# AnjieCheng/SpatialRGPT

Measured on NVIDIA H100. Metric: generated_tokens_per_sec, higher is better.
Workload: dtype bf16

## Files before the change

spatialrgpt_b200/csrc/gemv.cu:

```cuda
#include <stdlib.h>

#include "common.cuh"
#include "pack12.cuh"
#include "srgpt_b200.h"

namespace srgpt {
namespace gemv {

constexpr int THREADS = 256;
constexpr int WARPS = THREADS / 32;
constexpr int SPRE_MAX = 2;
constexpr int SPRE_WARP_BYTES = 2 * 4 * 32 * 16;
constexpr int SPRE_WARP_BYTES12 = 2 * 3 * 32 * 16;
enum { MODE_LM = 3 };

struct Params {
  const bf16* x;
  const bf16* W;
  int ldw;
  bf16* y;
  int N, K;
  const bf16* norm_weight;
  float eps;
  const bf16* residual;
  int n_heads, n_kv_heads, hd;
  const bf16* cos_tab;
  const bf16* sin_tab;
  const int* pos;
  bf16* kv_pages;
  const int* page_table;
  int page_size;
  float* logits_out;
  float* part_val;
  int* part_idx;
  unsigned long long* trace;
  int spre;
  int l2pf;
  int kv_heads_total;
  int kv_head_off;
  float* y_f32;
  srgpt_packed12 pk;
};

__device__ __forceinline__ void pdl_launch_dependents() { asm volatile("griddepcontrol.launch_dependents;" ::: "memory"); }
__device__ __forceinline__ void pdl_wait() { asm volatile("griddepcontrol.wait;" ::: "memory"); }

__device__ __forceinline__ void stage_x(const bf16* __restrict__ x, const bf16* __restrict__ norm_weight, float eps, int K,
                                        bf16* sx, float* red, const uint4* nw_pre, bool nw_pre_valid) {
  const int nchunk = K >> 3;
  if (norm_weight == nullptr) {
    for (int c = threadIdx.x; c < nchunk; c += THREADS)
      reinterpret_cast<uint4*>(sx)[c] = reinterpret_cast<const uint4*>(x)[c];
  } else if (nw_pre_valid) {
    uint4 xr[2];
    float sq = 0.f;
#pragma unroll
    for (int k = 0; k < 2; ++k) {
      const int c = threadIdx.x + k * THREADS;
      xr[k] = make_uint4(0, 0, 0, 0);
      if (c < nchunk) xr[k] = reinterpret_cast<const uint4*>(x)[c];
      float f[8];
      unpack8(xr[k], f);
#pragma unroll
      for (int t = 0; t < 8; ++t) sq += f[t] * f[t];
    }
    const float rstd = rsqrtf(block_sum(sq, red) / (float)K + eps);
#pragma unroll
    for (int k = 0; k < 2; ++k) {
      const int c = threadIdx.x + k * THREADS;
      if (c < nchunk) {
        float f[8], w[8], o[8];
        unpack8(xr[k], f);
        unpack8(nw_pre[k], w);
#pragma unroll
        for (int t = 0; t < 8; ++t) o[t] = w[t] * bf16_round(f[t] * rstd);
        reinterpret_cast<uint4*>(sx)[c] = pack8(o);
      }
    }
  } else {
    float sq = 0.f;
    for (int c = threadIdx.x; c < nchunk; c += THREADS) {
      float f[8];
      unpack8(reinterpret_cast<const uint4*>(x)[c], f);
#pragma unroll
      for (int t = 0; t < 8; ++t) sq += f[t] * f[t];
    }
    const float rstd = rsqrtf(block_sum(sq, red) / (float)K + eps);
    for (int c = threadIdx.x; c < nchunk; c += THREADS) {
      float f[8], w[8], o[8];
      unpack8(reinterpret_cast<const uint4*>(x)[c], f);
      unpack8(reinterpret_cast<const uint4*>(norm_weight)[c], w);
#pragma unroll
      for (int t = 0; t < 8; ++t) o[t] = w[t] * bf16_round(f[t] * rstd);
      reinterpret_cast<uint4*>(sx)[c] = pack8(o);
    }
  }
  __syncthreads();
}

__device__ __forceinline__ float dot8(const uint4& w, const float* xf) {
  float f[8];
  unpack8(w, f);
  float a = 0.f;
#pragma unroll
  for (int t = 0; t < 8; ++t) a = fmaf(f[t], xf[t], a);
  return a;
}

__device__ __forceinline__ bool better(float v, int i, float bv, int bi) { return v > bv || (v == bv && i < bi); }

template <int MODE>
__device__ __forceinline__ void pair_rows(const Params& p, int pi, int& r0, int& r1) {
  if (MODE == SRGPT_GEMV_QKV_ROPE) {
    const int half = p.hd >> 1;
    const int head = pi / half, j = pi - head * half;
    r0 = head * p.hd + j;
    r1 = r0 + half;
  } else {
    r0 = 2 * pi;
    r1 = r0 + 1;
    if (MODE == MODE_LM && r1 >= p.N) r1 = r0;
  }
}

struct Raw12 {
  uint4 s01, s23, e;
};

__device__ __forceinline__ Raw12 ld_raw12(const uint4* sm_lane, const uint4* ex_lane, int b) {
  Raw12 q;
  q.s01 = ld_stream16(sm_lane + b * 64);
  q.s23 = ld_stream16(sm_lane + b * 64 + 32);
  q.e = ld_stream16(ex_lane + b * 32);
  return q;
}

__device__ __forceinline__ void decode_batch(const Raw12& q, uint32_t bp, uint4 (&w)[4]) {
  w[0] = pack12::decode_chunk(q.s01.x, q.s01.y, q.e.x, bp);
  w[1] = pack12::decode_chunk(q.s01.z, q.s01.w, q.e.y, bp);
  w[2] = pack12::decode_chunk(q.s23.x, q.s23.y, q.e.z, bp);
  w[3] = pack12::decode_chunk(q.s23.z, q.s23.w, q.e.w, bp);
}

__device__ __forceinline__ void patch_batch(uint4 (&w)[4], int exc, int n, int& j, int b, int lane) {
  while (j < n) {
    const int v = __shfl_sync(0xffffffffu, exc, j);
    const int col = v >> 8;
    if ((col >> 10) != b) break;
    const int cc = col >> 3, t = col & 7;
    const uint32_t bits = ((cc & 31) == lane) ? (uint32_t)(v & 0xFF) << (7 + 16 * (t & 1)) : 0u;
#pragma unroll
    for (int i = 0; i < 4; ++i) {
      const uint32_t m = (i == ((cc >> 5) & 3)) ? bits : 0u;
      w[i].x |= (t >> 1) == 0 ? m : 0u;
      w[i].y |= (t >> 1) == 1 ? m : 0u;
      w[i].z |= (t >> 1) == 2 ? m : 0u;
      w[i].w |= (t >> 1) == 3 ? m : 0u;
    }
    ++j;
  }
}

struct Rows12 {
  uint32_t bp0, bp1;
  int exc0, exc1;
  int n0, n1;
  int j0, j1;
};

__device__ __forceinline__ void consume12(const Raw12& q0, const Raw12& q1, Rows12& rs, int b, int lane, const uint4* px, float& a0, float& a1) {
  uint4 w0[4], w1[4];
  decode_batch(q0, rs.bp0, w0);
  decode_batch(q1, rs.bp1, w1);
  patch_batch(w0, rs.exc0, rs.n0, rs.j0, b, lane);
  patch_batch(w1, rs.exc1, rs.n1, rs.j1, b, lane);
  const int c = b * 128 + lane;
#pragma unroll
  for (int i = 0; i < 4; ++i) {
    float xf[8];
    unpack8(px[c + 32 * i], xf);
    a0 += dot8(w0[i], xf);
    a1 += dot8(w1[i], xf);
  }
}

template <int MODE, int PRE, bool PACKED>
__global__ void __launch_bounds__(THREADS, PRE == 1 ? 3 : (PRE == 2 ? 2 : 1)) decode_gemv_kernel(const Params p) {
  extern __shared__ __align__(16) uint8_t smem_raw[];
  __shared__ float red[32];
  __shared__ float sv[WARPS];
  __shared__ int si[WARPS];
  bf16* sx = reinterpret_cast<bf16*>(smem_raw);

  const int warp = threadIdx.x >> 5, lane = threadIdx.x & 31;
  trace_mark(p.trace, 0);
  const int npairs = (MODE == MODE_LM) ? ((p.N + 1) >> 1) : (p.N >> 1);
  const int pi = blockIdx.x * WARPS + warp;
  const bool active = pi < npairs;
  int r0 = 0, r1 = 0;
  if (active) pair_rows<MODE>(p, pi, r0, r1);
  const uint4* p0 = reinterpret_cast<const uint4*>(p.W + (size_t)r0 * p.ldw);
  const uint4* p1 = reinterpret_cast<const uint4*>(p.W + (size_t)r1 * p.ldw);
  const uint4* px = reinterpret_cast<const uint4*>(sx);
  const int nchunk = p.K >> 3;
  const int nchunk_all = nchunk;

  constexpr int NPRE = 4 * PRE;
  uint4 u0[NPRE], u1[NPRE];
  int c = lane;
  const bool first_full = !PACKED && active && (c + 32 * (NPRE - 1) < nchunk);
  if (first_full) {
#pragma unroll
    for (int i = 0; i < NPRE; ++i) {
      u0[i] = ld_stream16(p0 + c + 32 * i);
      u1[i] = ld_stream16(p1 + c + 32 * i);
    }
  }
  uint8_t* spre_base = smem_raw + (size_t)p.K * 2 + (size_t)warp * ((size_t)p.spre * (PACKED ? SPRE_WARP_BYTES12 : SPRE_WARP_BYTES));
  int n_spre = 0;
  const int nbatch = p.K >> 10;
  Raw12 q0 = {}, q1 = {};
  Rows12 rs = {};
  const uint4 *sm0 = nullptr, *ex0 = nullptr;
  const int drow_ex = (r1 - r0) * (p.K >> 5);
  if (PACKED && active) {
    sm0 = reinterpret_cast<const uint4*>(p.pk.sm) + (size_t)r0 * (p.K >> 4) + lane;
    ex0 = reinterpret_cast<const uint4*>(p.pk.ex) + (size_t)r0 * (p.K >> 5) + lane;
    q0 = ld_raw12(sm0, ex0, 0);
    q1 = ld_raw12(sm0 + 2 * drow_ex, ex0 + drow_ex, 0);
    for (int b = 0; b < p.spre && 1 + b < nbatch; ++b) {
      const uint32_t d = (uint32_t)__cvta_generic_to_shared(spre_base + b * 6 * 512 + lane * 16);
      const uint4 *s = sm0 + (1 + b) * 64, *e = ex0 + (1 + b) * 32;
      asm volatile("cp.async.cg.shared.global [%0], [%1], 16;" ::"r"(d), "l"(s) : "memory");
      asm volatile("cp.async.cg.shared.global [%0], [%1], 16;" ::"r"(d + 512), "l"(s + 32) : "memory");
      asm volatile("cp.async.cg.shared.global [%0], [%1], 16;" ::"r"(d + 1024), "l"(e) : "memory");
      asm volatile("cp.async.cg.shared.global [%0], [%1], 16;" ::"r"(d + 1536), "l"(s + 2 * drow_ex) : "memory");
      asm volatile("cp.async.cg.shared.global [%0], [%1], 16;" ::"r"(d + 2048), "l"(s + 2 * drow_ex + 32) : "memory");
      asm volatile("cp.async.cg.shared.global [%0], [%1], 16;" ::"r"(d + 2560), "l"(e + drow_ex) : "memory");
      ++n_spre;
    }
    asm volatile("cp.async.commit_group;" ::: "memory");
    const int e0 = p.pk.row_ptr[r0], e1 = p.pk.row_ptr[r1];
    rs.n0 = min(p.pk.row_ptr[r0 + 1] - e0, pack12::MAX_EXC_PER_ROW);
    rs.n1 = min(p.pk.row_ptr[r1 + 1] - e1, pack12::MAX_EXC_PER_ROW);
    if (lane < rs.n0) rs.exc0 = p.pk.exc[e0 + lane];
    if (lane < rs.n1) rs.exc1 = p.pk.exc[e1 + lane];
    rs.bp0 = (uint32_t)p.pk.base[r0] - 1u;
    rs.bp1 = (uint32_t)p.pk.base[r1] - 1u;
  }
  if (first_full) {
    for (int b = 0; b < p.spre; ++b) {
      const int cb = c + 32 * NPRE + 128 * b;
      if (cb + 96 >= nchunk) break;
#pragma unroll
      for (int i = 0; i < 4; ++i) {
        const uint32_t d0 = (uint32_t)__cvta_generic_to_shared(spre_base + ((b * 2 + 0) * 4 + i) * 512 + lane * 16);
        const uint32_t d1 = (uint32_t)__cvta_generic_to_shared(spre_base + ((b * 2 + 1) * 4 + i) * 512 + lane * 16);
        asm volatile("cp.async.cg.shared.global [%0], [%1], 16;" ::"r"(d0), "l"(p0 + cb + 32 * i) : "memory");
        asm volatile("cp.async.cg.shared.global [%0], [%1], 16;" ::"r"(d1), "l"(p1 + cb + 32 * i) : "memory");
      }
      ++n_spre;
    }
    asm volatile("cp.async.commit_group;" ::: "memory");
  }
  if (!PACKED && p.l2pf && active && lane < 2) {
    const int c_req = first_full ? (32 * NPRE + 128 * n_spre) : 0;
    if (c_req < nchunk) {
      const char* rowp = reinterpret_cast<const char*>(lane == 0 ? p0 : p1) + (size_t)c_req * 16;
      uint32_t bytes = (uint32_t)(nchunk - c_req) * 16u;
      while (bytes > 0) {
        const uint32_t n = bytes > 16384u ? 16384u : bytes;
        asm volatile("cp.async.bulk.prefetch.L2.global [%0], %1;" ::"l"(rowp), "r"(n) : "memory");
        rowp += n;
        bytes -= n;
      }
    }
  }
  uint4 nw_pre[2] = {make_uint4(0, 0, 0, 0), make_uint4(0, 0, 0, 0)};
  const bool nw_pre_valid = (p.norm_weight != nullptr) && (nchunk_all <= 2 * THREADS);
  if (nw_pre_valid) {
#pragma unroll
    for (int k = 0; k < 2; ++k) {
      const int cc = threadIdx.x + k * THREADS;
      if (cc < nchunk_all) nw_pre[k] = reinterpret_cast<const uint4*>(p.norm_weight)[cc];
    }
  }
  pdl_launch_dependents();
  pdl_wait();
  trace_mark(p.trace, 1);

  stage_x(p.x, p.norm_weight, p.eps, p.K, sx, red, nw_pre, nw_pre_valid);

  float a0 = 0.f, a1 = 0.f;
  if constexpr (PACKED) {
    if (active) {
      consume12(q0, q1, rs, 0, lane, px, a0, a1);
      if (n_spre > 0) {
        asm volatile("cp.async.wait_group 0;" ::: "memory");
        for (int b = 0; b < n_spre; ++b) {
          const uint8_t* s = spre_base + b * 6 * 512 + lane * 16;
          const Raw12 t0 = {*reinterpret_cast<const uint4*>(s), *reinterpret_cast<const uint4*>(s + 512), *reinterpret_cast<const uint4*>(s + 1024)};
          const Raw12 t1 = {*reinterpret_cast<const uint4*>(s + 1536), *reinterpret_cast<const uint4*>(s + 2048), *reinterpret_cast<const uint4*>(s + 2560)};
          consume12(t0, t1, rs, 1 + b, lane, px, a0, a1);
        }
      }
      for (int b = 1 + n_spre; b < nbatch; ++b) {
        const Raw12 t0 = ld_raw12(sm0, ex0, b), t1 = ld_raw12(sm0 + 2 * drow_ex, ex0 + drow_ex, b);
        consume12(t0, t1, rs, b, lane, px, a0, a1);
      }
    }
  } else if (active) {
    if (first_full) {
#pragma unroll
      for (int i = 0; i < NPRE; ++i) {
        float xf[8];
        unpack8(px[c + 32 * i], xf);
        a0 += dot8(u0[i], xf);
        a1 += dot8(u1[i], xf);
      }
      c += 32 * NPRE;
      if (n_spre > 0) {
        asm volatile("cp.async.wait_group 0;" ::: "memory");
        for (int b = 0; b < n_spre; ++b) {
#pragma unroll
          for (int i = 0; i < 4; ++i) {
            float xf[8];
            unpack8(px[c + 32 * i], xf);
            const uint4 w0 = *reinterpret_cast<const uint4*>(spre_base + ((b * 2 + 0) * 4 + i) * 512 + lane * 16);
            const uint4 w1 = *reinterpret_cast<const uint4*>(spre_base + ((b * 2 + 1) * 4 + i) * 512 + lane * 16);
            a0 += dot8(w0, xf);
            a1 += dot8(w1, xf);
          }
          c += 128;
        }
      }
    }
    for (; c + 96 < nchunk; c += 128) {
#pragma unroll
      for (int i = 0; i < 4; ++i) {
        u0[i] = ld_stream16(p0 + c + 32 * i);
        u1[i] = ld_stream16(p1 + c + 32 * i);
      }
#pragma unroll
      for (int i = 0; i < 4; ++i) {
        float xf[8];
        unpack8(px[c + 32 * i], xf);
        a0 += dot8(u0[i], xf);
        a1 += dot8(u1[i], xf);
      }
    }
    for (; c < nchunk; c += 32) {
      float xf[8];
      unpack8(px[c], xf);
      a0 += dot8(ld_stream16(p0 + c), xf);
      a1 += dot8(ld_stream16(p1 + c), xf);
    }
  }
  a0 = warp_sum(a0);
  a1 = warp_sum(a1);
  float best = -INFINITY;
  int besti = 0x7fffffff;
  if (active && lane == 0) {
    if (MODE == SRGPT_GEMV_PLAIN && p.y_f32 != nullptr) {
      *reinterpret_cast<float2*>(p.y_f32 + r0) = make_float2(a0, a1);
    } else if (MODE == SRGPT_GEMV_PLAIN) {
      float y0 = bf16_round(a0), y1 = bf16_round(a1);
      if (p.residual != nullptr) {
        y0 += e2f(p.residual[r0]);
        y1 += e2f(p.residual[r1]);
      }
      *reinterpret_cast<uint32_t*>(p.y + r0) = pack_bf16x2(y0, y1);
    } else if (MODE == SRGPT_GEMV_SWIGLU) {
      const float g = bf16_round(a0), u = bf16_round(a1);
      p.y[pi] = f2e(bf16_round(silu(g)) * u);
    } else if (MODE == SRGPT_GEMV_QKV_ROPE) {
      const int half = p.hd >> 1;
      const int head = pi / half, j = pi - head * half;
      float v0 = bf16_round(a0), v1 = bf16_round(a1);
      const int pos = *p.pos;
      if (head < p.n_heads + p.n_kv_heads) {
        const float cs = e2f(p.cos_tab[(size_t)pos * half + j]);
        const float sn = e2f(p.sin_tab[(size_t)pos * half + j]);
        const float o0 = bf16_round(bf16_round(v0 * cs) + bf16_round(-v1 * sn));
        const float o1 = bf16_round(bf16_round(v1 * cs) + bf16_round(v0 * sn));
        v0 = o0;
        v1 = o1;
      }
      if (head < p.n_heads) {
        p.y[r0] = f2e(v0);
        p.y[r1] = f2e(v1);
      } else {
        const int page = p.page_table[pos / p.page_size], slot = pos % p.page_size;
        const bool is_v = head >= p.n_heads + p.n_kv_heads;
        const int kh = head - p.n_heads - (is_v ? p.n_kv_heads : 0) + p.kv_head_off;
        const int kv_row = (p.kv_heads_total > 0 ? p.kv_heads_total : p.n_kv_heads) * p.hd;
        bf16* dst = p.kv_pages + (((size_t)page * 2 + (is_v ? 1 : 0)) * p.page_size + slot) * kv_row + kh * p.hd;
        dst[j] = f2e(v0);
        dst[j + half] = f2e(v1);
      }
    } else {
      a0 = bf16_round(a0);
      a1 = bf16_round(a1);
      if (p.logits_out != nullptr) {
        p.logits_out[r0] = a0;
        if (r1 != r0) p.logits_out[r1] = a1;
      }
      best = a0;
      besti = r0;
      if (r1 != r0 && better(a1, r1, best, besti)) { best = a1; besti = r1; }
    }
  }
  if (MODE == MODE_LM) {
    if (lane == 0) { sv[warp] = best; si[warp] = besti; }
    __syncthreads();
    if (threadIdx.x == 0) {
      for (int w = 1; w < WARPS; ++w)
        if (better(sv[w], si[w], best, besti)) { best = sv[w]; besti = si[w]; }
      p.part_val[blockIdx.x] = best;
      p.part_idx[blockIdx.x] = besti;
    }
  }
  trace_mark(p.trace, 2);
}

__global__ void __launch_bounds__(256)
lm_head_finalize_kernel(const float* __restrict__ part_val, const int* __restrict__ part_idx, int nparts,
                        const bf16* __restrict__ embed_table, bf16* __restrict__ next_x, int K, long long* __restrict__ out_ids,
                        int* step, int* pos) {
  __shared__ float sv[8];
  __shared__ int si[8];
  __shared__ int s_tok;
  pdl_launch_dependents();
  pdl_wait();
  float best = -INFINITY;
  int bi = 0x7fffffff;
  for (int i = threadIdx.x; i < nparts; i += blockDim.x)
    if (better(part_val[i], part_idx[i], best, bi)) { best = part_val[i]; bi = part_idx[i]; }
#pragma unroll
  for (int o = 16; o > 0; o >>= 1) {
    const float ov = __shfl_xor_sync(0xffffffffu, best, o);
    const int oi = __shfl_xor_sync(0xffffffffu, bi, o);
    if (better(ov, oi, best, bi)) { best = ov; bi = oi; }
  }
  if ((threadIdx.x & 31) == 0) { sv[threadIdx.x >> 5] = best; si[threadIdx.x >> 5] = bi; }
  __syncthreads();
  if (threadIdx.x == 0) {
    for (int w = 1; w < 8; ++w)
      if (better(sv[w], si[w], best, bi)) { best = sv[w]; bi = si[w]; }
    if (bi == 0x7fffffff) bi = 0;
    s_tok = bi;
    out_ids[*step] = (long long)bi;
  }
  __syncthreads();
  const int tok = s_tok;
  if (embed_table != nullptr && next_x != nullptr) {
    const uint4* src = reinterpret_cast<const uint4*>(embed_table + (size_t)tok * K);
    for (int c = threadIdx.x; c < (K >> 3); c += blockDim.x) reinterpret_cast<uint4*>(next_x)[c] = src[c];
  }
  __syncthreads();
  if (threadIdx.x == 0) {
    *step += 1;
    *pos += 1;
  }
}

constexpr int MT_MAX = SRGPT_SPEC_T_MAX;
constexpr int MT_TILE_CH = 512;

struct MParams {
  Params p;
  int T;
  int ldx, ldy;
  int tile_ch;
};

template <int MODE, bool PACKED>
__global__ void __launch_bounds__(THREADS, 2) decode_gemv_multi_kernel(const MParams mp) {
  extern __shared__ __align__(16) uint8_t smem_raw[];
  __shared__ float red[32];
  __shared__ float sv[MT_MAX][WARPS];
  __shared__ int si[MT_MAX][WARPS];
  const Params& p = mp.p;
  const int nt = mp.T, tile_ch = mp.tile_ch;
  bf16* sx = reinterpret_cast<bf16*>(smem_raw);
  const uint4* px = reinterpret_cast<const uint4*>(sx);

  const int warp = threadIdx.x >> 5, lane = threadIdx.x & 31;
  const int npairs = (MODE == MODE_LM) ? ((p.N + 1) >> 1) : (p.N >> 1);
  const int pi = blockIdx.x * WARPS + warp;
  const bool active = pi < npairs;
  int r0 = 0, r1 = 0;
  if (active) pair_rows<MODE>(p, pi, r0, r1);
  const int nchunk = p.K >> 3;
  const int nbatch = (nchunk + 127) >> 7;

  const uint4* p0 = reinterpret_cast<const uint4*>(p.W + (size_t)r0 * p.ldw);
  const uint4* p1 = reinterpret_cast<const uint4*>(p.W + (size_t)r1 * p.ldw);
  uint4 u0[4], u1[4];
  Raw12 q0 = {}, q1 = {};
  Rows12 rs = {};
  const uint4 *sm0 = nullptr, *ex0 = nullptr;
  const int drow_ex = (r1 - r0) * (p.K >> 5);
  auto load_plain = [&](int b, uint4 (&w0)[4], uint4 (&w1)[4]) {
#pragma unroll
    for (int i = 0; i < 4; ++i) {
      const int c = b * 128 + lane + 32 * i;
      w0[i] = make_uint4(0, 0, 0, 0);
      w1[i] = make_uint4(0, 0, 0, 0);
      if (c < nchunk) {
        w0[i] = ld_stream16(p0 + c);
        w1[i] = ld_stream16(p1 + c);
      }
    }
  };
  if (active) {
    if constexpr (PACKED) {
      sm0 = reinterpret_cast<const uint4*>(p.pk.sm) + (size_t)r0 * (p.K >> 4) + lane;
      ex0 = reinterpret_cast<const uint4*>(p.pk.ex) + (size_t)r0 * (p.K >> 5) + lane;
      q0 = ld_raw12(sm0, ex0, 0);
      q1 = ld_raw12(sm0 + 2 * drow_ex, ex0 + drow_ex, 0);
      const int e0 = p.pk.row_ptr[r0], e1 = p.pk.row_ptr[r1];
      rs.n0 = min(p.pk.row_ptr[r0 + 1] - e0, pack12::MAX_EXC_PER_ROW);
      rs.n1 = min(p.pk.row_ptr[r1 + 1] - e1, pack12::MAX_EXC_PER_ROW);
      if (lane < rs.n0) rs.exc0 = p.pk.exc[e0 + lane];
      if (lane < rs.n1) rs.exc1 = p.pk.exc[e1 + lane];
      rs.bp0 = (uint32_t)p.pk.base[r0] - 1u;
      rs.bp1 = (uint32_t)p.pk.base[r1] - 1u;
    } else {
      load_plain(0, u0, u1);
    }
  }
  uint4 nw_pre[2] = {make_uint4(0, 0, 0, 0), make_uint4(0, 0, 0, 0)};
  const bool nw_pre_valid = (p.norm_weight != nullptr) && (nchunk <= 2 * THREADS);
  if (nw_pre_valid) {
#pragma unroll
    for (int k = 0; k < 2; ++k) {
      const int cc = threadIdx.x + k * THREADS;
      if (cc < nchunk) nw_pre[k] = reinterpret_cast<const uint4*>(p.norm_weight)[cc];
    }
  }
  pdl_launch_dependents();
  pdl_wait();

  float a0[MT_MAX], a1[MT_MAX];
#pragma unroll
  for (int t = 0; t < MT_MAX; ++t) a0[t] = a1[t] = 0.f;
  int b = 0;
  for (int c0 = 0; c0 < nchunk; c0 += tile_ch) {
    const int tlen = min(tile_ch, nchunk - c0);
    if (p.norm_weight != nullptr) {
      for (int t = 0; t < nt; ++t)
        stage_x(p.x + (size_t)t * mp.ldx, p.norm_weight, p.eps, p.K, sx + (size_t)t * tile_ch * 8, red, nw_pre, nw_pre_valid);
    } else {
      __syncthreads();
      for (int t = 0; t < nt; ++t) {
        const uint4* src = reinterpret_cast<const uint4*>(p.x + (size_t)t * mp.ldx) + c0;
        uint4* dst = reinterpret_cast<uint4*>(sx) + (size_t)t * tile_ch;
        for (int cc = threadIdx.x; cc < tlen; cc += THREADS) dst[cc] = src[cc];
      }
      __syncthreads();
    }
    if (!active) continue;
    for (; b < nbatch && b * 128 < c0 + tlen; ++b) {
      uint4 w0[4], w1[4];
      if constexpr (PACKED) {
        if (b > 0) {
          q0 = ld_raw12(sm0, ex0, b);
          q1 = ld_raw12(sm0 + 2 * drow_ex, ex0 + drow_ex, b);
        }
        decode_batch(q0, rs.bp0, w0);
        decode_batch(q1, rs.bp1, w1);
        patch_batch(w0, rs.exc0, rs.n0, rs.j0, b, lane);
        patch_batch(w1, rs.exc1, rs.n1, rs.j1, b, lane);
      } else {
        if (b > 0) load_plain(b, u0, u1);
#pragma unroll
        for (int i = 0; i < 4; ++i) {
          w0[i] = u0[i];
          w1[i] = u1[i];
        }
      }
#pragma unroll
      for (int i = 0; i < 4; ++i) {
        const int c = b * 128 + lane + 32 * i;
        if (c < nchunk) {
#pragma unroll
          for (int t = 0; t < MT_MAX; ++t) {
            if (t < nt) {
              float xf[8];
              unpack8(px[(size_t)t * tile_ch + (c - c0)], xf);
              a0[t] += dot8(w0[i], xf);
              a1[t] += dot8(w1[i], xf);
            }
          }
        }
      }
    }
  }
#pragma unroll
  for (int t = 0; t < MT_MAX; ++t) {
    if (t < nt) {
      a0[t] = warp_sum(a0[t]);
      a1[t] = warp_sum(a1[t]);
    }
  }
  float s0 = 0.f, s1 = 0.f;
#pragma unroll
  for (int t = 0; t < MT_MAX; ++t) {
    if (t == lane) {
      s0 = a0[t];
      s1 = a1[t];
    }
  }
  if (active && lane < nt) {
    {
      const int t = lane;
      bf16* y = p.y + (size_t)t * mp.ldy;
      if (MODE == SRGPT_GEMV_PLAIN) {
        float y0 = bf16_round(s0), y1 = bf16_round(s1);
        if (p.residual != nullptr) {
          const bf16* res = p.residual + (size_t)t * mp.ldy;
          y0 += e2f(res[r0]);
          y1 += e2f(res[r1]);
        }
        *reinterpret_cast<uint32_t*>(y + r0) = pack_bf16x2(y0, y1);
      } else if (MODE == SRGPT_GEMV_SWIGLU) {
        const float g = bf16_round(s0), u = bf16_round(s1);
        y[pi] = f2e(bf16_round(silu(g)) * u);
      } else if (MODE == SRGPT_GEMV_QKV_ROPE) {
        const int half = p.hd >> 1;
        const int head = pi / half, j = pi - head * half;
        float v0 = bf16_round(s0), v1 = bf16_round(s1);
        const int pos = *p.pos + t;
        if (head < p.n_heads + p.n_kv_heads) {
          const float cs = e2f(p.cos_tab[(size_t)pos * half + j]);
          const float sn = e2f(p.sin_tab[(size_t)pos * half + j]);
          const float o0 = bf16_round(bf16_round(v0 * cs) + bf16_round(-v1 * sn));
          const float o1 = bf16_round(bf16_round(v1 * cs) + bf16_round(v0 * sn));
          v0 = o0;
          v1 = o1;
        }
        if (head < p.n_heads) {
          y[r0] = f2e(v0);
          y[r1] = f2e(v1);
        } else {
          const int page = p.page_table[pos / p.page_size], slot = pos % p.page_size;
          const bool is_v = head >= p.n_heads + p.n_kv_heads;
          const int kh = head - p.n_heads - (is_v ? p.n_kv_heads : 0);
          bf16* dst = p.kv_pages + (((size_t)page * 2 + (is_v ? 1 : 0)) * p.page_size + slot) * ((size_t)p.n_kv_heads * p.hd) + kh * p.hd;
          dst[j] = f2e(v0);
          dst[j + half] = f2e(v1);
        }
      } else {
        const float l0 = bf16_round(s0), l1 = bf16_round(s1);
        if (p.logits_out != nullptr) {
          float* lo = p.logits_out + (size_t)t * p.N;
          lo[r0] = l0;
          if (r1 != r0) lo[r1] = l1;
        }
        float best = l0;
        int besti = r0;
        if (r1 != r0 && better(l1, r1, best, besti)) { best = l1; besti = r1; }
        sv[t][warp] = best;
        si[t][warp] = besti;
      }
    }
  }
  if (MODE == MODE_LM) {
    if (!active && lane < nt) {
      sv[lane][warp] = -INFINITY;
      si[lane][warp] = 0x7fffffff;
    }
    __syncthreads();
    if (threadIdx.x < nt) {
      const int t = threadIdx.x;
      float best = sv[t][0];
      int besti = si[t][0];
      for (int w = 1; w < WARPS; ++w)
        if (better(sv[t][w], si[t][w], best, besti)) { best = sv[t][w]; besti = si[t][w]; }
      float* pv = p.part_val + (size_t)t * 2 * gridDim.x;
      pv[blockIdx.x] = best;
      reinterpret_cast<int*>(pv + gridDim.x)[blockIdx.x] = besti;
    }
  }
}

struct SpecHist {
  const int* prompt;
  int P;
  const long long* out;
  __device__ __forceinline__ int operator()(int i) const { return i < P ? prompt[i] : (int)out[i - P]; }
};

__global__ void __launch_bounds__(256)
spec_draft_kernel(const int* __restrict__ prompt_ids, const int* __restrict__ prompt_len, const long long* __restrict__ out_ids, const int* __restrict__ step,
                  const int* __restrict__ pos, int* __restrict__ pos_rows, int T, int ngram, const bf16* __restrict__ embed_table,
                  bf16* __restrict__ x, int H, int* __restrict__ draft_ids, int* __restrict__ state) {
  __shared__ int s_min[8];
  __shared__ int s_draft[MT_MAX];
  const int P = prompt_len != nullptr ? *prompt_len : 0;
  const SpecHist hist{prompt_ids, P, out_ids};
  const int s = *step, L = P + s;
  int start = -1;
  for (int n = min(ngram, L - 1); n >= 1 && start < 0; --n) {
    int best = 0x7fffffff;
    for (int i = threadIdx.x; i < L - n; i += blockDim.x) {
      bool eq = true;
      for (int j = 0; j < n && eq; ++j) {
        const int v = hist(i + j);
        eq = v >= 0 && v == hist(L - n + j);
      }
      if (eq) { best = i; break; }
    }
#pragma unroll
    for (int o = 16; o > 0; o >>= 1) best = min(best, __shfl_xor_sync(0xffffffffu, best, o));
    if ((threadIdx.x & 31) == 0) s_min[threadIdx.x >> 5] = best;
    __syncthreads();
    int m = 0x7fffffff;
    for (int w = 0; w < (int)(blockDim.x >> 5); ++w) m = min(m, s_min[w]);
    __syncthreads();
    if (m != 0x7fffffff) start = m + n;
  }
  if (threadIdx.x == 0) {
    int nd = 0;
    s_draft[0] = hist(L - 1);
    for (int t = 1; t < T; ++t) {
      int v = -1;
      if (start >= 0 && nd == t - 1 && start + t - 1 < L) {
        v = hist(start + t - 1);
        if (v >= 0) ++nd; else v = -1;
      }
      s_draft[t] = v;
    }
    state[3] = nd;
  }
  __syncthreads();
  if (threadIdx.x < T) {
    draft_ids[threadIdx.x] = s_draft[threadIdx.x];
    pos_rows[threadIdx.x] = *pos + (int)threadIdx.x;
  }
  for (int t = 0; t < T; ++t) {
    const uint4* src = reinterpret_cast<const uint4*>(embed_table + (size_t)max(s_draft[t], 0) * H);
    uint4* dst = reinterpret_cast<uint4*>(x + (size_t)t * H);
    for (int c = threadIdx.x; c < (H >> 3); c += blockDim.x) dst[c] = src[c];
  }
}

__global__ void __launch_bounds__(256)
spec_accept_kernel(const float* __restrict__ ws, int nparts, int T, const int* __restrict__ draft_ids, long long* __restrict__ out_ids, int out_cap,
                   int* step, int* pos, int* state) {
  __shared__ float sv[8];
  __shared__ int si[8];
  __shared__ int s_tok[MT_MAX];
  pdl_launch_dependents();
  pdl_wait();
  for (int t = 0; t < T; ++t) {
    const float* part_val = ws + (size_t)t * 2 * nparts;
    const int* part_idx = reinterpret_cast<const int*>(part_val + nparts);
    float best = -INFINITY;
    int bi = 0x7fffffff;
    for (int i = threadIdx.x; i < nparts; i += blockDim.x)
      if (better(part_val[i], part_idx[i], best, bi)) { best = part_val[i]; bi = part_idx[i]; }
#pragma unroll
    for (int o = 16; o > 0; o >>= 1) {
      const float ov = __shfl_xor_sync(0xffffffffu, best, o);
      const int oi = __shfl_xor_sync(0xffffffffu, bi, o);
      if (better(ov, oi, best, bi)) { best = ov; bi = oi; }
    }
    if ((threadIdx.x & 31) == 0) { sv[threadIdx.x >> 5] = best; si[threadIdx.x >> 5] = bi; }
    __syncthreads();
    if (threadIdx.x == 0) {
      for (int w = 1; w < 8; ++w)
        if (better(sv[w], si[w], best, bi)) { best = sv[w]; bi = si[w]; }
      if (bi == 0x7fffffff) bi = 0;
      s_tok[t] = bi;
    }
    __syncthreads();
  }
  if (threadIdx.x == 0) {
    int a = 0;
    while (a < T - 1 && draft_ids[a + 1] == s_tok[a]) ++a;
    const int s0 = *step;
    for (int t = 0; t <= a; ++t)
      if (s0 + t < out_cap) out_ids[s0 + t] = (long long)s_tok[t];
    state[0] += 1;
    state[1] += state[3];
    state[2] += a;
    state[4] = s0;
    state[5] = a + 1;
    state[6] = s0 + a + 1;
    *step = s0 + a + 1;
    *pos += a + 1;
  }
}

__global__ void __launch_bounds__(256) spec_copy_logits_kernel(const float* __restrict__ rows, float* __restrict__ all, int V, const int* __restrict__ state,
                                                               int out_cap) {
  const int t = blockIdx.y;
  if (t >= state[5] || state[4] + t >= out_cap) return;
  const float* src = rows + (size_t)t * V;
  float* dst = all + (size_t)(state[4] + t) * V;
  for (int j = blockIdx.x * blockDim.x + threadIdx.x; j < V; j += gridDim.x * blockDim.x) dst[j] = src[j];
}

__global__ void __launch_bounds__(256)
lm_head_local_best_kernel(const float* __restrict__ part_val, const int* __restrict__ part_idx, int nparts, int index_base, int* __restrict__ best) {
  __shared__ float sv[8];
  __shared__ int si[8];
  pdl_launch_dependents();
  pdl_wait();
  float bv = -INFINITY;
  int bi = 0x7fffffff;
  for (int i = threadIdx.x; i < nparts; i += blockDim.x)
    if (better(part_val[i], part_idx[i], bv, bi)) { bv = part_val[i]; bi = part_idx[i]; }
#pragma unroll
  for (int o = 16; o > 0; o >>= 1) {
    const float ov = __shfl_xor_sync(0xffffffffu, bv, o);
    const int oi = __shfl_xor_sync(0xffffffffu, bi, o);
    if (better(ov, oi, bv, bi)) { bv = ov; bi = oi; }
  }
  if ((threadIdx.x & 31) == 0) { sv[threadIdx.x >> 5] = bv; si[threadIdx.x >> 5] = bi; }
  __syncthreads();
  if (threadIdx.x == 0) {
    for (int w = 1; w < 8; ++w)
      if (better(sv[w], si[w], bv, bi)) { bv = sv[w]; bi = si[w]; }
    best[0] = __float_as_int(bv);
    best[1] = (bi == 0x7fffffff) ? index_base : bi + index_base;
  }
}

__global__ void __launch_bounds__(256)
tp_pick_token_kernel(const int* __restrict__ best_all, int world, const bf16* __restrict__ embed_table, bf16* __restrict__ next_x, int K,
                     long long* __restrict__ out_ids, int* step, int* pos) {
  __shared__ int s_tok;
  if (threadIdx.x == 0) {
    float bv = -INFINITY;
    int bi = 0x7fffffff;
    for (int r = 0; r < world; ++r) {
      const float v = __int_as_float(best_all[2 * r]);
      const int i = best_all[2 * r + 1];
      if (better(v, i, bv, bi)) { bv = v; bi = i; }
    }
    if (bi == 0x7fffffff) bi = 0;
    s_tok = bi;
    out_ids[*step] = (long long)bi;
  }
  __syncthreads();
  const int tok = s_tok;
  if (embed_table != nullptr && next_x != nullptr) {
    const uint4* src = reinterpret_cast<const uint4*>(embed_table + (size_t)tok * K);
    for (int c = threadIdx.x; c < (K >> 3); c += blockDim.x) reinterpret_cast<uint4*>(next_x)[c] = src[c];
  }
  __syncthreads();
  if (threadIdx.x == 0) {
    *step += 1;
    *pos += 1;
  }
}

__global__ void __launch_bounds__(256) tp_residual_add_kernel(bf16* __restrict__ h, const float* __restrict__ partial, int n) {
  const int i = blockIdx.x * blockDim.x + threadIdx.x;
  if (i < n) h[i] = f2e(bf16_round(partial[i]) + e2f(h[i]));
}

static int grid_for(int npairs) { return ceil_div(npairs, WARPS); }

static void pdl_config(cudaLaunchConfig_t& cfg, cudaLaunchAttribute* attr, int grid, int block, int smem, cudaStream_t st) {
  cfg = {};
  cfg.gridDim = dim3(grid);
  cfg.blockDim = dim3(block);
  cfg.dynamicSmemBytes = smem;
  cfg.stream = st;
  attr[0].id = cudaLaunchAttributeProgrammaticStreamSerialization;
  attr[0].val.programmaticStreamSerializationAllowed = 1;
  cfg.attrs = attr;
  cfg.numAttrs = pdl_enabled() ? 1 : 0;
}

static int spre_default() {
  static const int v = [] {
    const char* e = getenv("SRGPT_GEMV_SPRE");
    const int x = (e != nullptr && e[0] != 0) ? atoi(e) : 1;
    return x < 0 ? 0 : (x > SPRE_MAX ? SPRE_MAX : x);
  }();
  return v;
}

template <int MODE, int PRE, bool PACKED = false>
static int launch_pre(const Params& p, int npairs, cudaStream_t st) {
  const int smem = p.K * 2 + WARPS * spre_default() * (PACKED ? SPRE_WARP_BYTES12 : SPRE_WARP_BYTES);
  static int configured_smem = 0;
  if (smem > 48 * 1024 && smem > configured_smem) {
    SRGPT_CHECK_CUDA(cudaFuncSetAttribute(decode_gemv_kernel<MODE, PRE, PACKED>, cudaFuncAttributeMaxDynamicSharedMemorySize, smem));
    configured_smem = smem;
  }
  cudaLaunchConfig_t cfg;
  cudaLaunchAttribute attr[1];
  pdl_config(cfg, attr, grid_for(npairs), THREADS, smem, st);
  Params q = p;
  q.trace = trace_next_slot();
  q.spre = spre_default();
  static const int l2pf = [] {
    const char* v = getenv("SRGPT_GEMV_L2PF");
    return (v != nullptr && v[0] != 0) ? atoi(v) : 0;
  }();
  const bool small_plain = MODE == SRGPT_GEMV_PLAIN && p.residual != nullptr && (long long)p.N * p.K <= (32LL << 20);
  q.l2pf = (l2pf == 1 || (l2pf >= 2 && small_plain) || (l2pf == 3 && MODE == SRGPT_GEMV_QKV_ROPE)) ? 1 : 0;
  SRGPT_CHECK_CUDA(cudaLaunchKernelEx(&cfg, decode_gemv_kernel<MODE, PRE, PACKED>, q));
  return SRGPT_OK;
}

template <int MODE>
static int launch(const Params& p, int npairs, cudaStream_t st) {
  static const int pre_small = [] {
    const char* v = getenv("SRGPT_GEMV_PRE_SMALL");
    const int x = (v != nullptr && v[0] != 0) ? atoi(v) : 1;
    return (x == 1 || x == 2 || x == 4) ? x : 1;
  }();
  const bool small = (MODE == SRGPT_GEMV_PLAIN || MODE == SRGPT_GEMV_QKV_ROPE) && ((size_t)p.N * p.K * 2 <= (size_t)64 << 20);
  if (small && pre_small == 4 && (p.K >> 3) >= 512) return launch_pre<MODE, 4>(p, npairs, st);
  if (small && pre_small >= 2 && (p.K >> 3) >= 256) return launch_pre<MODE, 2>(p, npairs, st);
  return launch_pre<MODE, 1>(p, npairs, st);
}

template <int MODE, bool PACKED>
static int launch_mode(const Params& p, int npairs, cudaStream_t st) {
  if constexpr (PACKED) return launch_pre<MODE, 1, true>(p, npairs, st);
  else return launch<MODE>(p, npairs, st);
}

}
}

using namespace srgpt;

static bool aligned16(const void* p) { return (reinterpret_cast<uintptr_t>(p) & 15) == 0; }

static bool packed_ok(const srgpt_packed12* P, int K) {
  return P != nullptr && P->sm && P->ex && P->base && P->row_ptr && P->exc && aligned16(P->sm) && aligned16(P->ex) && (K % pack12::BATCH) == 0;
}

template <bool PACKED>
static int gemv_modes(gemv::Params& p, const void* x, void* y, int N, int K, const void* norm_weight, float eps, const void* residual, int mode,
                      int n_heads, int n_kv_heads, int head_dim, const void* cos_tab, const void* sin_tab, const int* pos, void* kv_pages,
                      const int* page_table, int page_size, void* stream) {
  SRGPT_CHECK_ARG(x && y && N > 0 && K > 0);
  SRGPT_CHECK_ARG((N % 2) == 0 && (K % 8) == 0);
  SRGPT_CHECK_ARG(K * 2 <= 200 * 1024);
  SRGPT_CHECK_ARG(aligned16(x) && (reinterpret_cast<uintptr_t>(y) & 3) == 0);
  SRGPT_CHECK_ARG(norm_weight == nullptr || aligned16(norm_weight));
  SRGPT_CHECK_ARG(mode >= SRGPT_GEMV_PLAIN && mode <= SRGPT_GEMV_QKV_ROPE);
  SRGPT_CHECK_ARG(x != y);
  p.x = reinterpret_cast<const bf16*>(x);
  p.y = reinterpret_cast<bf16*>(y);
  p.N = N; p.K = K;
  p.norm_weight = reinterpret_cast<const bf16*>(norm_weight);
  p.eps = eps;
  p.residual = reinterpret_cast<const bf16*>(residual);
  p.n_heads = n_heads; p.n_kv_heads = n_kv_heads; p.hd = head_dim;
  p.cos_tab = reinterpret_cast<const bf16*>(cos_tab);
  p.sin_tab = reinterpret_cast<const bf16*>(sin_tab);
  p.pos = pos;
  p.kv_pages = reinterpret_cast<bf16*>(kv_pages);
  p.page_table = page_table;
  p.page_size = page_size;
  cudaStream_t st = reinterpret_cast<cudaStream_t>(stream);
  switch (mode) {
    case SRGPT_GEMV_PLAIN:
      p.hd = 2;
      return gemv::launch_mode<SRGPT_GEMV_PLAIN, PACKED>(p, N / 2, st);
    case SRGPT_GEMV_SWIGLU:
      SRGPT_CHECK_ARG(residual == nullptr);
      p.hd = 2;
      return gemv::launch_mode<SRGPT_GEMV_SWIGLU, PACKED>(p, N / 2, st);
    case SRGPT_GEMV_QKV_ROPE:
      SRGPT_CHECK_ARG(residual == nullptr && n_heads > 0 && n_kv_heads > 0 && head_dim > 0 && (head_dim % 2) == 0);
      SRGPT_CHECK_ARG(N == (n_heads + 2 * n_kv_heads) * head_dim);
      SRGPT_CHECK_ARG(cos_tab && sin_tab && pos && kv_pages && page_table && page_size > 0);
      return gemv::launch_mode<SRGPT_GEMV_QKV_ROPE, PACKED>(p, N / 2, st);
  }
  return SRGPT_ERR_INVALID;
}

extern "C" __attribute__((visibility("default"))) int srgpt_gemv_bf16(const void* x, const void* W, int ldw, void* y, int N, int K, const void* norm_weight, float eps,
                               const void* residual, int mode, int n_heads, int n_kv_heads, int head_dim, const void* cos_tab,
                               const void* sin_tab, const int* pos, void* kv_pages, const int* page_table, int page_size,
                               void* stream) {
  SRGPT_CHECK_ARG(W && aligned16(W) && (ldw % 8) == 0 && ldw >= K);
  gemv::Params p = {};
  p.W = reinterpret_cast<const bf16*>(W);
  p.ldw = ldw;
  return gemv_modes<false>(p, x, y, N, K, norm_weight, eps, residual, mode, n_heads, n_kv_heads, head_dim, cos_tab, sin_tab, pos, kv_pages,
                           page_table, page_size, stream);
}

extern "C" __attribute__((visibility("default"))) int srgpt_gemv_packed_bf16(const void* x, const srgpt_packed12* packed, void* y, int N, int K,
                                                                               const void* norm_weight, float eps, const void* residual, int mode, int n_heads,
                                                                               int n_kv_heads, int head_dim, const void* cos_tab, const void* sin_tab,
                                                                               const int* pos, void* kv_pages, const int* page_table, int page_size,
                                                                               void* stream) {
  SRGPT_CHECK_ARG(packed_ok(packed, K));
#ifdef SRGPT_ELEM_F16
  set_last_error("srgpt_gemv_packed_bf16: the 12-bit packing is defined for bfloat16 weights only");
  return SRGPT_ERR_UNSUPPORTED;
#else
  gemv::Params p = {};
  p.pk = *packed;
  return gemv_modes<true>(p, x, y, N, K, norm_weight, eps, residual, mode, n_heads, n_kv_heads, head_dim, cos_tab, sin_tab, pos, kv_pages,
                          page_table, page_size, stream);
#endif
}

extern "C" __attribute__((visibility("default"))) int srgpt_gemv_tp_bf16(const void* x, const void* W, int ldw, void* y, int N, int K, const void* norm_weight, float eps,
                                                                         int mode, int n_heads, int n_kv_heads, int head_dim, const void* cos_tab, const void* sin_tab,
                                                                         const int* pos, void* kv_pages, const int* page_table, int page_size, int kv_heads_total,
                                                                         int kv_head_off, float* partial_f32, void* stream) {
  SRGPT_CHECK_ARG(x && W && N > 0 && K > 0 && (y != nullptr || partial_f32 != nullptr));
  SRGPT_CHECK_ARG((N % 2) == 0 && (K % 8) == 0 && (ldw % 8) == 0 && ldw >= K && K * 2 <= 200 * 1024);
  SRGPT_CHECK_ARG(aligned16(x) && aligned16(W) && (norm_weight == nullptr || aligned16(norm_weight)));
  SRGPT_CHECK_ARG(mode == SRGPT_GEMV_PLAIN || mode == SRGPT_GEMV_QKV_ROPE);
  gemv::Params p = {};
  p.x = reinterpret_cast<const bf16*>(x);
  p.W = reinterpret_cast<const bf16*>(W);
  p.ldw = ldw;
  p.y = reinterpret_cast<bf16*>(y);
  p.N = N; p.K = K;
  p.norm_weight = reinterpret_cast<const bf16*>(norm_weight);
  p.eps = eps;
  cudaStream_t st = reinterpret_cast<cudaStream_t>(stream);
  if (mode == SRGPT_GEMV_PLAIN) {
    SRGPT_CHECK_ARG(partial_f32 != nullptr && (reinterpret_cast<uintptr_t>(partial_f32) & 7) == 0);
    p.hd = 2;
    p.y_f32 = partial_f32;
    return gemv::launch<SRGPT_GEMV_PLAIN>(p, N / 2, st);
  }
  SRGPT_CHECK_ARG(y != nullptr && (reinterpret_cast<uintptr_t>(y) & 3) == 0 && x != y);
  SRGPT_CHECK_ARG(n_heads > 0 && n_kv_heads > 0 && head_dim > 0 && (head_dim % 2) == 0 && N == (n_heads + 2 * n_kv_heads) * head_dim);
  SRGPT_CHECK_ARG(cos_tab && sin_tab && pos && kv_pages && page_table && page_size > 0);
  SRGPT_CHECK_ARG(kv_heads_total >= n_kv_heads && kv_head_off >= 0 && kv_head_off + n_kv_heads <= kv_heads_total);
  p.n_heads = n_heads; p.n_kv_heads = n_kv_heads; p.hd = head_dim;
  p.cos_tab = reinterpret_cast<const bf16*>(cos_tab);
  p.sin_tab = reinterpret_cast<const bf16*>(sin_tab);
  p.pos = pos;
  p.kv_pages = reinterpret_cast<bf16*>(kv_pages);
  p.page_table = page_table;
  p.page_size = page_size;
  p.kv_heads_total = kv_heads_total;
  p.kv_head_off = kv_head_off;
  return gemv::launch<SRGPT_GEMV_QKV_ROPE>(p, N / 2, st);
}

extern "C" __attribute__((visibility("default"))) int srgpt_tp_residual_add_bf16(void* h, const float* partial, int n, void* stream) {
  SRGPT_CHECK_ARG(h && partial && n > 0);
  gemv::tp_residual_add_kernel<<<ceil_div(n, 256), 256, 0, reinterpret_cast<cudaStream_t>(stream)>>>(reinterpret_cast<bf16*>(h), partial, n);
  SRGPT_CHECK_LAUNCH();
  return SRGPT_OK;
}

extern "C" __attribute__((visibility("default"))) int srgpt_lm_head_local_best_bf16(const void* x, const void* W_local, int ldw, int V_local, int K, const void* norm_weight,
                                                                                    float eps, void* workspace, int index_base, int* best, void* stream) {
  SRGPT_CHECK_ARG(x && W_local && workspace && best && V_local > 0 && K > 0 && index_base >= 0);
  SRGPT_CHECK_ARG((K % 8) == 0 && (ldw % 8) == 0 && ldw >= K && K * 2 <= 200 * 1024);
  SRGPT_CHECK_ARG(aligned16(x) && aligned16(W_local) && (norm_weight == nullptr || aligned16(norm_weight)));
  const int npairs = (V_local + 1) / 2;
  const int g = gemv::grid_for(npairs);
  gemv::Params p = {};
  p.x = reinterpret_cast<const bf16*>(x);
  p.W = reinterpret_cast<const bf16*>(W_local);
  p.ldw = ldw; p.N = V_local; p.K = K;
  p.norm_weight = reinterpret_cast<const bf16*>(norm_weight);
  p.eps = eps;
  p.hd = 2;
  p.part_val = reinterpret_cast<float*>(workspace);
  p.part_idx = reinterpret_cast<int*>(p.part_val + g);
  cudaStream_t st = reinterpret_cast<cudaStream_t>(stream);
  int rc = gemv::launch<gemv::MODE_LM>(p, npairs, st);
  if (rc != SRGPT_OK) return rc;
  cudaLaunchConfig_t cfg;
  cudaLaunchAttribute attr[1];
  gemv::pdl_config(cfg, attr, 1, 256, 0, st);
  SRGPT_CHECK_CUDA(cudaLaunchKernelEx(&cfg, gemv::lm_head_local_best_kernel, (const float*)p.part_val, (const int*)p.part_idx, g, index_base, best));
  return SRGPT_OK;
}

extern "C" __attribute__((visibility("default"))) int srgpt_tp_pick_token(const int* best_all, int world, const void* embed_table, void* next_x, int K, long long* out_ids,
                                                                          int* step, int* pos, void* stream) {
  SRGPT_CHECK_ARG(best_all && world > 0 && out_ids && step && pos);
  SRGPT_CHECK_ARG((embed_table == nullptr) == (next_x == nullptr));
  SRGPT_CHECK_ARG(embed_table == nullptr || ((K % 8) == 0 && aligned16(embed_table) && aligned16(next_x)));
  gemv::tp_pick_token_kernel<<<1, 256, 0, reinterpret_cast<cudaStream_t>(stream)>>>(best_all, world, reinterpret_cast<const bf16*>(embed_table),
                                                                                  reinterpret_cast<bf16*>(next_x), K, out_ids, step, pos);
  SRGPT_CHECK_LAUNCH();
  return SRGPT_OK;
}

extern "C" __attribute__((visibility("default"))) long long srgpt_lm_head_workspace(int V) {
  if (V <= 0) return -1;
  const int g = gemv::grid_for((V + 1) / 2);
  return (long long)g * (long long)(sizeof(float) + sizeof(int));
}

template <bool PACKED>
static int lm_head_argmax(gemv::Params& p, const void* x, int V, int K, const void* norm_weight, float eps, float* logits_out, void* workspace,
                          const void* embed_table, void* next_x, long long* out_ids, int* step, int* pos, void* stream) {
  SRGPT_CHECK_ARG(x && workspace && out_ids && step && pos && V > 0 && K > 0);
  SRGPT_CHECK_ARG((K % 8) == 0 && K * 2 <= 200 * 1024);
  SRGPT_CHECK_ARG(aligned16(x) && (norm_weight == nullptr || aligned16(norm_weight)));
  SRGPT_CHECK_ARG((embed_table == nullptr) == (next_x == nullptr));
  SRGPT_CHECK_ARG(embed_table == nullptr || (aligned16(embed_table) && aligned16(next_x)));
  const int npairs = (V + 1) / 2;
  const int g = gemv::grid_for(npairs);
  p.x = reinterpret_cast<const bf16*>(x);
  p.N = V; p.K = K;
  p.norm_weight = reinterpret_cast<const bf16*>(norm_weight);
  p.eps = eps;
  p.hd = 2;
  p.logits_out = logits_out;
  p.part_val = reinterpret_cast<float*>(workspace);
  p.part_idx = reinterpret_cast<int*>(p.part_val + g);
  cudaStream_t st = reinterpret_cast<cudaStream_t>(stream);
  int rc = gemv::launch_mode<gemv::MODE_LM, PACKED>(p, npairs, st);
  if (rc != SRGPT_OK) return rc;
  cudaLaunchConfig_t cfg;
  cudaLaunchAttribute attr[1];
  gemv::pdl_config(cfg, attr, 1, 256, 0, st);
  SRGPT_CHECK_CUDA(cudaLaunchKernelEx(&cfg, gemv::lm_head_finalize_kernel, (const float*)p.part_val, (const int*)p.part_idx, g,
                                      reinterpret_cast<const bf16*>(embed_table), reinterpret_cast<bf16*>(next_x), K, out_ids, step, pos));
  return SRGPT_OK;
}

extern "C" __attribute__((visibility("default"))) int srgpt_lm_head_argmax_bf16(const void* x, const void* W, int ldw, int V, int K, const void* norm_weight, float eps,
                                         float* logits_out, void* workspace, const void* embed_table, void* next_x,
                                         long long* out_ids, int* step, int* pos, void* stream) {
  SRGPT_CHECK_ARG(W && aligned16(W) && (ldw % 8) == 0 && ldw >= K);
  gemv::Params p = {};
  p.W = reinterpret_cast<const bf16*>(W);
  p.ldw = ldw;
  return lm_head_argmax<false>(p, x, V, K, norm_weight, eps, logits_out, workspace, embed_table, next_x, out_ids, step, pos, stream);
}

extern "C" __attribute__((visibility("default"))) int srgpt_lm_head_argmax_packed_bf16(const void* x, const srgpt_packed12* packed, int V, int K,
                                                                                         const void* norm_weight, float eps, float* logits_out, void* workspace,
                                                                                         const void* embed_table, void* next_x, long long* out_ids, int* step,
                                                                                         int* pos, void* stream) {
  SRGPT_CHECK_ARG(packed_ok(packed, K));
#ifdef SRGPT_ELEM_F16
  set_last_error("srgpt_lm_head_argmax_packed_bf16: the 12-bit packing is defined for bfloat16 weights only");
  return SRGPT_ERR_UNSUPPORTED;
#else
  gemv::Params p = {};
  p.pk = *packed;
  return lm_head_argmax<true>(p, x, V, K, norm_weight, eps, logits_out, workspace, embed_table, next_x, out_ids, step, pos, stream);
#endif
}

namespace srgpt {
namespace gemv {

template <int MODE, bool PACKED>
static int launch_multi(MParams& mp, int npairs, cudaStream_t st) {
  const int smem = mp.T * mp.tile_ch * 16;
  static int configured_smem = 0;
  if (smem > configured_smem) {
    SRGPT_CHECK_CUDA(cudaFuncSetAttribute(decode_gemv_multi_kernel<MODE, PACKED>, cudaFuncAttributeMaxDynamicSharedMemorySize, smem));
    configured_smem = smem;
  }
  cudaLaunchConfig_t cfg;
  cudaLaunchAttribute attr[1];
  pdl_config(cfg, attr, grid_for(npairs), THREADS, smem, st);
  SRGPT_CHECK_CUDA(cudaLaunchKernelEx(&cfg, decode_gemv_multi_kernel<MODE, PACKED>, mp));
  return SRGPT_OK;
}

static int multi_tile(int K, bool norm) { return norm ? (K >> 3) : ((K >> 3) < MT_TILE_CH ? (K >> 3) : MT_TILE_CH); }

}
}

template <bool PACKED>
static int gemv_multi_modes(gemv::MParams& mp, const void* x, int ldx, void* y, int ldy, int T, int N, int K, const void* norm_weight, float eps,
                            const void* residual, int mode, int n_heads, int n_kv_heads, int head_dim, const void* cos_tab, const void* sin_tab,
                            const int* pos, void* kv_pages, const int* page_table, int page_size, void* stream) {
  SRGPT_CHECK_ARG(x && y && N > 0 && K > 0 && T >= 1 && T <= gemv::MT_MAX);
  SRGPT_CHECK_ARG((N % 2) == 0 && (K % 8) == 0 && (ldx % 8) == 0 && ldx >= K && (ldy % 2) == 0);
  SRGPT_CHECK_ARG(aligned16(x) && (reinterpret_cast<uintptr_t>(y) & 3) == 0);
  SRGPT_CHECK_ARG(norm_weight == nullptr || aligned16(norm_weight));
  SRGPT_CHECK_ARG(mode >= SRGPT_GEMV_PLAIN && mode <= SRGPT_GEMV_QKV_ROPE);
  SRGPT_CHECK_ARG(x != y);
  const int tile = gemv::multi_tile(K, norm_weight != nullptr);
  SRGPT_CHECK_ARG(T * tile * 16 <= 200 * 1024);
  gemv::Params& p = mp.p;
  p.x = reinterpret_cast<const bf16*>(x);
  p.y = reinterpret_cast<bf16*>(y);
  p.N = N; p.K = K;
  p.norm_weight = reinterpret_cast<const bf16*>(norm_weight);
  p.eps = eps;
  p.residual = reinterpret_cast<const bf16*>(residual);
  p.n_heads = n_heads; p.n_kv_heads = n_kv_heads; p.hd = head_dim;
  p.cos_tab = reinterpret_cast<const bf16*>(cos_tab);
  p.sin_tab = reinterpret_cast<const bf16*>(sin_tab);
  p.pos = pos;
  p.kv_pages = reinterpret_cast<bf16*>(kv_pages);
  p.page_table = page_table;
  p.page_size = page_size;
// ... 122 lines not shown
```

Measured before the change: 183.5.

## Stream packed 12-bit GEMV weights through a cp.async ring buffer

In the packed 12-bit GEMV path, each prefetch batch now gets its own cp.async commit group. A per-warp shared-memory ring, two slots deep by default, is refilled with batch b+depth right after batch b is read from its slot, so weight loads stay in flight for the whole K loop instead of only the first few batches. The ring depth is set by an env var and capped by the number of batches, and it replaces the old SPRE-based shared-memory sizing for packed kernels. The risk is extra wait_group and shared-memory round trips that may not beat the plain direct loads in a bandwidth-bound kernel.

```diff
diff --git a/spatialrgpt_b200/csrc/gemv.cu b/spatialrgpt_b200/csrc/gemv.cu
--- a/spatialrgpt_b200/csrc/gemv.cu
+++ b/spatialrgpt_b200/csrc/gemv.cu
@@ -30,6 +30,7 @@
   bf16* kv_pages;
   const int* page_table;
   int page_size;
+  int ring;
   float* logits_out;
   float* part_val;
   int* part_idx;
@@ -158,6 +159,33 @@
       w[i].w |= (t >> 1) == 3 ? m : 0u;
     }
     ++j;
+  }
+}
+
+__device__ __forceinline__ void cp_async_batch12(const uint8_t* slot_lane, const uint4* sm0, const uint4* ex0, int drow_ex, int b) {
+  const uint32_t d = (uint32_t)__cvta_generic_to_shared(slot_lane);
+  const uint4 *s = sm0 + b * 64, *e = ex0 + b * 32;
+  asm volatile("cp.async.cg.shared.global [%0], [%1], 16;" ::"r"(d), "l"(s) : "memory");
+  asm volatile("cp.async.cg.shared.global [%0], [%1], 16;" ::"r"(d + 512), "l"(s + 32) : "memory");
+  asm volatile("cp.async.cg.shared.global [%0], [%1], 16;" ::"r"(d + 1024), "l"(e) : "memory");
+  asm volatile("cp.async.cg.shared.global [%0], [%1], 16;" ::"r"(d + 1536), "l"(s + 2 * drow_ex) : "memory");
+  asm volatile("cp.async.cg.shared.global [%0], [%1], 16;" ::"r"(d + 2048), "l"(s + 2 * drow_ex + 32) : "memory");
+  asm volatile("cp.async.cg.shared.global [%0], [%1], 16;" ::"r"(d + 2560), "l"(e + drow_ex) : "memory");
+}
+
+__device__ __forceinline__ void ld_slot12(const uint8_t* slot_lane, Raw12& t0, Raw12& t1) {
+  const uint4* s = reinterpret_cast<const uint4*>(slot_lane);
+  t0 = {s[0], s[32], s[64]};
+  t1 = {s[96], s[128], s[160]};
+}
+
+constexpr int RING_MAX = 4;
+__device__ __forceinline__ void cp_async_wait_pending(int n) {
+  switch (n) {
+    case 0: asm volatile("cp.async.wait_group 0;" ::: "memory"); break;
+    case 1: asm volatile("cp.async.wait_group 1;" ::: "memory"); break;
+    case 2: asm volatile("cp.async.wait_group 2;" ::: "memory"); break;
+    default: asm volatile("cp.async.wait_group 3;" ::: "memory"); break;
   }
 }
 
@@ -229,17 +257,10 @@
     q0 = ld_raw12(sm0, ex0, 0);
     q1 = ld_raw12(sm0 + 2 * drow_ex, ex0 + drow_ex, 0);
     for (int b = 0; b < p.spre && 1 + b < nbatch; ++b) {
-      const uint32_t d = (uint32_t)__cvta_generic_to_shared(spre_base + b * 6 * 512 + lane * 16);
-      const uint4 *s = sm0 + (1 + b) * 64, *e = ex0 + (1 + b) * 32;
-      asm volatile("cp.async.cg.shared.global [%0], [%1], 16;" ::"r"(d), "l"(s) : "memory");
-      asm volatile("cp.async.cg.shared.global [%0], [%1], 16;" ::"r"(d + 512), "l"(s + 32) : "memory");
-      asm volatile("cp.async.cg.shared.global [%0], [%1], 16;" ::"r"(d + 1024), "l"(e) : "memory");
-      asm volatile("cp.async.cg.shared.global [%0], [%1], 16;" ::"r"(d + 1536), "l"(s + 2 * drow_ex) : "memory");
-      asm volatile("cp.async.cg.shared.global [%0], [%1], 16;" ::"r"(d + 2048), "l"(s + 2 * drow_ex + 32) : "memory");
-      asm volatile("cp.async.cg.shared.global [%0], [%1], 16;" ::"r"(d + 2560), "l"(e + drow_ex) : "memory");
+      cp_async_batch12(spre_base + b * SPRE_WARP_BYTES12 + lane * 16, sm0, ex0, drow_ex, 1 + b);
+      asm volatile("cp.async.commit_group;" ::: "memory");
       ++n_spre;
     }
-    asm volatile("cp.async.commit_group;" ::: "memory");
     const int e0 = p.pk.row_ptr[r0], e1 = p.pk.row_ptr[r1];
     rs.n0 = min(p.pk.row_ptr[r0 + 1] - e0, pack12::MAX_EXC_PER_ROW);
     rs.n1 = min(p.pk.row_ptr[r1 + 1] - e1, pack12::MAX_EXC_PER_ROW);
@@ -295,18 +316,33 @@
   if constexpr (PACKED) {
     if (active) {
       consume12(q0, q1, rs, 0, lane, px, a0, a1);
-      if (n_spre > 0) {
-        asm volatile("cp.async.wait_group 0;" ::: "memory");
-        for (int b = 0; b < n_spre; ++b) {
-          const uint8_t* s = spre_base + b * 6 * 512 + lane * 16;
-          const Raw12 t0 = {*reinterpret_cast<const uint4*>(s), *reinterpret_cast<const uint4*>(s + 512), *reinterpret_cast<const uint4*>(s + 1024)};
-          const Raw12 t1 = {*reinterpret_cast<const uint4*>(s + 1536), *reinterpret_cast<const uint4*>(s + 2048), *reinterpret_cast<const uint4*>(s + 2560)};
-          consume12(t0, t1, rs, 1 + b, lane, px, a0, a1);
+      if (p.ring) {
+        int slot = 0;
+        for (int b = 1; b < nbatch; ++b) {
+          cp_async_wait_pending(min(n_spre - 1, nbatch - 1 - b));
+          const uint8_t* s = spre_base + slot * SPRE_WARP_BYTES12 + lane * 16;
+          Raw12 t0, t1;
+          ld_slot12(s, t0, t1);
+          if (b + n_spre < nbatch) {
+            cp_async_batch12(s, sm0, ex0, drow_ex, b + n_spre);
+            asm volatile("cp.async.commit_group;" ::: "memory");
+          }
+          consume12(t0, t1, rs, b, lane, px, a0, a1);
+          if (++slot == n_spre) slot = 0;
         }
-      }
-      for (int b = 1 + n_spre; b < nbatch; ++b) {
-        const Raw12 t0 = ld_raw12(sm0, ex0, b), t1 = ld_raw12(sm0 + 2 * drow_ex, ex0 + drow_ex, b);
-        consume12(t0, t1, rs, b, lane, px, a0, a1);
+      } else {
+        if (n_spre > 0) {
+          asm volatile("cp.async.wait_group 0;" ::: "memory");
+          for (int b = 0; b < n_spre; ++b) {
+            Raw12 t0, t1;
+            ld_slot12(spre_base + b * SPRE_WARP_BYTES12 + lane * 16, t0, t1);
+            consume12(t0, t1, rs, 1 + b, lane, px, a0, a1);
+          }
+        }
+        for (int b = 1 + n_spre; b < nbatch; ++b) {
+          const Raw12 t0 = ld_raw12(sm0, ex0, b), t1 = ld_raw12(sm0 + 2 * drow_ex, ex0 + drow_ex, b);
+          consume12(t0, t1, rs, b, lane, px, a0, a1);
+        }
       }
     }
   } else if (active) {
@@ -886,9 +922,20 @@
   return v;
 }
 
+static int ring_depth(int K) {
+  const char* e = getenv("SRGPT_GEMV_RING");
+  int d = (e != nullptr && e[0] != 0) ? atoi(e) : 2;
+  if (d <= 0) return -1;
+  d = d > RING_MAX ? RING_MAX : d;
+  const int later = (K >> 10) - 1;
+  return d < later ? d : later;
+}
+
 template <int MODE, int PRE, bool PACKED = false>
 static int launch_pre(const Params& p, int npairs, cudaStream_t st) {
-  const int smem = p.K * 2 + WARPS * spre_default() * (PACKED ? SPRE_WARP_BYTES12 : SPRE_WARP_BYTES);
+  const int ring = PACKED ? ring_depth(p.K) : -1;
+  const int spre = ring >= 0 ? ring : spre_default();
+  const int smem = p.K * 2 + WARPS * spre * (PACKED ? SPRE_WARP_BYTES12 : SPRE_WARP_BYTES);
   static int configured_smem = 0;
   if (smem > 48 * 1024 && smem > configured_smem) {
     SRGPT_CHECK_CUDA(cudaFuncSetAttribute(decode_gemv_kernel<MODE, PRE, PACKED>, cudaFuncAttributeMaxDynamicSharedMemorySize, smem));
@@ -899,7 +946,8 @@
   pdl_config(cfg, attr, grid_for(npairs), THREADS, smem, st);
   Params q = p;
   q.trace = trace_next_slot();
-  q.spre = spre_default();
+  q.spre = spre;
+  q.ring = ring >= 0 ? 1 : 0;
   static const int l2pf = [] {
     const char* v = getenv("SRGPT_GEMV_L2PF");
     return (v != nullptr && v[0] != 0) ? atoi(v) : 0;
```

Result: faster. 191.8, median of 6 (+4.5%).
